# JacobPorter/FastNeighborNet

Measured on AMD Instinct MI355X. Metric: sec to circular order, n=32768 taxa (+ achieved HBM GB/s), lower is better.
Workload: dtype f64

## Files before the change

fastneighbornet_amd/csrc/fnn_hip.hip:

```cpp
#include <hip/hip_runtime.h>

#include <dlfcn.h>

#include <cmath>
#include <limits>
#include <new>

#include "fnn_chain.h"
#include "fnn_engine.h"

namespace fnn {

struct fnn_nccl_id { char internal[FNN_COMM_ID_BYTES]; };

constexpr int SCAN_TW = 512;
constexpr int SCAN_TH = 32;
constexpr int SCAN_THREADS = 256;

static_assert(sizeof(Cand) == 24, "rec_publish / rec_fetch move a Cand as three 8-byte words");
__device__ inline uint64_t rec_check_word(const Cand& c, uint32_t tag) {
    return __builtin_bit_cast(uint64_t, c.q) ^ (c.key * 0x9E3779B97F4A7C15ULL) ^
           ((uint64_t)(uint32_t)c.si | ((uint64_t)(uint32_t)c.sj << 32)) ^ (((uint64_t)tag + 1ULL) * 0xBF58476D1CE4E5B9ULL);
}
__device__ inline void rec_publish(Cand* p, const Cand& c, uint64_t* chk, uint32_t tag) {
    __hip_atomic_store(chk, rec_check_word(c, tag), __ATOMIC_RELAXED, __HIP_MEMORY_SCOPE_AGENT);
    uint64_t* w = (uint64_t*)p;
    __hip_atomic_store(w + 0, __builtin_bit_cast(uint64_t, c.q), __ATOMIC_RELAXED, __HIP_MEMORY_SCOPE_AGENT);
    __hip_atomic_store(w + 1, c.key, __ATOMIC_RELAXED, __HIP_MEMORY_SCOPE_AGENT);
    __hip_atomic_store(w + 2, (uint64_t)(uint32_t)c.si | ((uint64_t)(uint32_t)c.sj << 32), __ATOMIC_RELAXED, __HIP_MEMORY_SCOPE_AGENT);
}
__device__ inline Cand rec_fetch(const Cand* p) {
    uint64_t* w = (uint64_t*)p;
    const uint64_t a = __hip_atomic_load(w + 0, __ATOMIC_RELAXED, __HIP_MEMORY_SCOPE_AGENT);
    const uint64_t b = __hip_atomic_load(w + 1, __ATOMIC_RELAXED, __HIP_MEMORY_SCOPE_AGENT);
    const uint64_t x = __hip_atomic_load(w + 2, __ATOMIC_RELAXED, __HIP_MEMORY_SCOPE_AGENT);
    Cand c;
    c.q = __builtin_bit_cast(double, a);
    c.key = b;
    c.si = (int)(uint32_t)x;
    c.sj = (int)(uint32_t)(x >> 32);
    return c;
}

template <int CTRL, int ROW_MASK>
__device__ __forceinline__ void dpp_pull(double q, uint64_t key, double& oq, uint64_t& ok) {
    const uint64_t qb = __builtin_bit_cast(uint64_t, q);
    const int ql = (int)(uint32_t)qb, qh = (int)(uint32_t)(qb >> 32), kl = (int)(uint32_t)key, kh = (int)(uint32_t)(key >> 32);
    const uint32_t oql = (uint32_t)__builtin_amdgcn_update_dpp(ql, ql, CTRL, ROW_MASK, 0xf, false);
    const uint32_t oqh = (uint32_t)__builtin_amdgcn_update_dpp(qh, qh, CTRL, ROW_MASK, 0xf, false);
    const uint32_t okl = (uint32_t)__builtin_amdgcn_update_dpp(kl, kl, CTRL, ROW_MASK, 0xf, false);
    const uint32_t okh = (uint32_t)__builtin_amdgcn_update_dpp(kh, kh, CTRL, ROW_MASK, 0xf, false);
    oq = __builtin_bit_cast(double, ((uint64_t)oqh << 32) | oql);
    ok = ((uint64_t)okh << 32) | okl;
}
__device__ __forceinline__ Cand wave_reduce(Cand c) {
    double q = c.q;
    uint64_t key = c.key;
#define FNN_DPP_STEP(CTRL, MASK) do { double oq; uint64_t ok; dpp_pull<CTRL, MASK>(q, key, oq, ok); \
        if (oq < q || (oq == q && ok < key)) { q = oq; key = ok; } } while (0)
    FNN_DPP_STEP(0x111, 0xf);
    FNN_DPP_STEP(0x112, 0xf);
    FNN_DPP_STEP(0x114, 0xf);
    FNN_DPP_STEP(0x118, 0xf);
    FNN_DPP_STEP(0x142, 0xa);
    FNN_DPP_STEP(0x143, 0xc);
#undef FNN_DPP_STEP
    Cand r;
    const uint64_t qb = __builtin_bit_cast(uint64_t, q);
    const uint32_t rql = (uint32_t)__builtin_amdgcn_readlane((int)(uint32_t)qb, 63), rqh = (uint32_t)__builtin_amdgcn_readlane((int)(uint32_t)(qb >> 32), 63);
    const uint32_t rkl = (uint32_t)__builtin_amdgcn_readlane((int)(uint32_t)key, 63), rkh = (uint32_t)__builtin_amdgcn_readlane((int)(uint32_t)(key >> 32), 63);
    r.q = __builtin_bit_cast(double, ((uint64_t)rqh << 32) | rql);
    r.key = ((uint64_t)rkh << 32) | rkl;
    const unsigned long long src = __ballot(c.key == r.key);
    const int l = src ? (int)__builtin_ctzll(src) : 0;
    r.si = __builtin_amdgcn_readlane(c.si, l);
    r.sj = __builtin_amdgcn_readlane(c.sj, l);
    return r;
}

template <int NWAVES>
__device__ __forceinline__ Cand block_reduce(Cand c, Cand* sh) {
    c = wave_reduce(c);
    int lane = threadIdx.x & 63, w = threadIdx.x >> 6;
    if (lane == 0) sh[w] = c;
    __syncthreads();
    if (threadIdx.x == 0) {
#pragma unroll
        for (int k = 1; k < NWAVES; k++)
            if (cand_better(sh[k], c)) c = sh[k];
    }
    return c;
}

constexpr int SCAN_R = SCAN_TW / SCAN_TH;

// ... 1895 lines not shown
            rl_rowmin_block(d, L);
            if (threadIdx.x == 0) rl_publish_part(d, L, seq);
        }
        return;
    }
    if (threadIdx.x < 64) {
        RlBlockEnv env{L, (int)threadIdx.x};
        const Cand out = relaxed_find(d, env);
        if (threadIdx.x == 0) {
            d.recs[0] = out;
            L.cmd = 2;
            if (gridDim.x > 1) st_sc1(d.rl_mail, rl_cmd_word(stamp, L.seq + 1u, RL_EXIT));
        }
        if (ticks && threadIdx.x == 0) {
            d.ticks[24] += L.tk[0]; d.ticks[25] += L.tk[1]; d.ticks[26] += (long long)wall_clock64() - tstart; d.ticks[27] += L.tk[3];
        }
        __syncthreads();
    } else {
        for (;;) {
            __syncthreads();
            if (L.cmd == 2) break;
            rl_rowmin_block(d, L);
        }
    }
}

template <bool HELP>
__global__ __launch_bounds__(CH_T) void k_decide(Dev d, const Cand* src, int nrecs, unsigned jobtag) {
    __shared__ ChainLds<CH_EPT> L;
    __shared__ DecideLds S;
    __shared__ Cand shc[CH_T / 64];
    __shared__ unsigned hword;
    State* st = d.st;
    if (HELP && blockIdx.x > 0) {
        rx_helper_workgroup(d, L, (int)blockIdx.x - 1, jobtag, &hword);
        return;
    }
    if (st->stall || st->la_hit) {
        if (HELP && threadIdx.x == 0) job_post(d, jobtag, 0u);
        return;
    }
    state_in(S.lst, st);
    if (threadIdx.x == 0) S.tkon = 0;
    Cand best = reduce_records(d, src, st->rl_active ? 1 : nrecs, shc);
    __syncthreads();
    decide_step<HELP, false>(d, S, L, best, jobtag);
    __syncthreads();
    if (threadIdx.x == 0) S.lst.rl_active = 0;
    __syncthreads();
    state_out(st, S.lst);
}

constexpr int TRK_THREADS = 1024;
constexpr int TRK_GROUP = 16;
constexpr int TRK_FLAG = 32 * 65;
constexpr int TRK_BAD = 32 * 67;

__device__ __forceinline__ void chain_workgroup(const Dev& d, ChainLds<CH_EPT>& L) {
    State* st = d.st;
    if (!st->chain_pending) return;
    const int32_t cU = st->chain_U, cm = st->chain_m;
    const unsigned evtag = (unsigned)st->n_events;
    const double usx = block_chain_sum2<CH_EPT>(d.chain, cm, CH_GUARD_BITS, L, nullptr);
    if (threadIdx.x == 0) {
        __hip_atomic_store(reinterpret_cast<uint64_t*>(d.Sx + cU), __builtin_bit_cast(uint64_t, usx), __ATOMIC_RELAXED, __HIP_MEMORY_SCOPE_AGENT);
        __hip_atomic_store(reinterpret_cast<uint64_t*>(d.Sx + cU + 1), __builtin_bit_cast(uint64_t, usx), __ATOMIC_RELAXED, __HIP_MEMORY_SCOPE_AGENT);
        __hip_atomic_store(reinterpret_cast<uint64_t*>(&upre_behind_ticket(d)->usx), __builtin_bit_cast(uint64_t, usx), __ATOMIC_RELAXED, __HIP_MEMORY_SCOPE_AGENT);
        asm volatile("s_waitcnt vmcnt(0)" ::: "memory");
        __hip_atomic_store(d.ticket + TRK_FLAG, evtag, __ATOMIC_RELAXED, __HIP_MEMORY_SCOPE_AGENT);
    }
}

__device__ __forceinline__ void sweep_exact_item(const Dev& d, int64_t r, const TrackArgs& ta, Cand& bx) {
    const int32_t half = (ta.m + 1) / 2;
    const int32_t fi = ta.nf0 + (int32_t)(r / half), cp = (int32_t)(r % half);
    if (fi >= ta.nf) return;
    const int32_t f0 = fresh_slot(d, fi, ta.m);
    if (f0 < 0) return;
    const int32_t s2 = 2 * cp;
    if (s2 >= ta.m || s2 == f0) return;
    const double* F0 = d.D + (int64_t)f0 * d.ld + s2;
    const double* F1 = F0 + d.ld;
    const double a0 = F0[0], a1 = F0[1], b0 = F1[0], b1 = F1[1];
    if (f0 > s2)
        scan_micro(f0, s2, ta.m, ta.twoP, ta.cm2, a0, a1, b0, b1, d.Sx[f0], d.Sx[f0 + 1], d.spos[f0], d.spos[f0 + 1],
                   d.Sx[s2], d.Sx[s2 + 1], d.spos[s2], d.spos[s2 + 1], bx);
    else
        scan_micro(s2, f0, ta.m, ta.twoP, ta.cm2, a0, b0, a1, b1, d.Sx[s2], d.Sx[s2 + 1], d.spos[s2], d.spos[s2 + 1],
                   d.Sx[f0], d.Sx[f0 + 1], d.spos[f0], d.spos[f0 + 1], bx);
}

constexpr int TRK_REC_U = 1024;

struct SpecialOut { double val, tu, tv; };
__device__ __forceinline__ SpecialOut special_wave(const Dev& d, const State& lst, double* blk, double* sxl, double* tl, int32_t* berr, double* chain_dst) {
    const int lane = threadIdx.x & 63;
    const int nS = __builtin_amdgcn_readfirstlane(lst.nS);
    const int32_t Sl = lane < nS ? lst.S[lane < MAX_S ? lane : 0] : -1;
    const int m_old = __builtin_amdgcn_readfirstlane(lst.m_old), twoP_old = 2 * __builtin_amdgcn_readfirstlane(lst.P_old);
    const int m = __builtin_amdgcn_readfirstlane(lst.m), twoP = 2 * __builtin_amdgcn_readfirstlane(lst.P);
    const int xs = __builtin_amdgcn_readfirstlane(lst.xs), ys = __builtin_amdgcn_readfirstlane(lst.ys);
    const int U = __builtin_amdgcn_readfirstlane(lst.U), V = U + 1;
    const int nops = __builtin_amdgcn_readfirstlane(lst.nops), ev_finish = __builtin_amdgcn_readfirstlane(lst.ev_finish);
    const int32_t myspos = (Sl >= 0 && Sl < m) ? d.spos[Sl] : 0;
    auto ixu = [&](int slot) -> int {
        const unsigned long long b = __ballot(Sl == slot && Sl >= 0);
        return b ? (int)__builtin_ctzll(b) : -1;
    };
    auto ixl = [&](int32_t slot) -> int {
        int r = -1;
#pragma unroll
        for (int j = 0; j < MAX_S; j++) if (__builtin_amdgcn_readlane(Sl, j) == slot && slot >= 0) r = j;
        return r;
    };
    const int me = lane;
    const int pold = (Sl >= 0 && Sl < twoP_old) ? ixl(Sl ^ 1) : -1;
    const int pnew = (Sl >= 0 && Sl < twoP && !(Sl & 1)) ? ixl(Sl + 1) : -1;
    auto B = [&](int r, int c) -> double& { return blk[r * MAX_S + c]; };
    auto bad = [&]() { *berr = 13; };
    SpecialOut out{0.0, 0.0, 0.0};
    if (!ev_finish) {
        const bool sp = Sl >= 0 && Sl < twoP_old;
        const bool act = Sl >= 0 && Sl < m_old && Sl != xs && Sl != ys && !(sp && (Sl & 1));
        double sx = 0.0, sxn = 0.0, told0 = 0.0, told1 = 0.0;
        bool bystander = true;
        if (act) { sx = sxl[me]; if (sp) { if (pold < 0) bad(); else sxn = sxl[pold]; } }
#pragma unroll
        for (int q = 0; q < 2; q++) {
            const int t = q == 0 ? xs : ys;
            const int tn = t < twoP_old ? (t ^ 1) : -1;
            const int it = ixu(t), itn = tn >= 0 ? ixu(tn) : -1;
            if (it < 0 || (tn >= 0 && itn < 0)) { bad(); continue; }
            if (!act) continue;
            if (Sl == t || Sl == tn) { bystander = false; continue; }
            double v;
            if (!sp && tn < 0) { const double e = B(it, me); v = e; told0 += e; }
            else if (sp && tn < 0) { const double e0 = B(it, me), e1 = B(it, pold); v = (e0 + e1) / 2.0; told0 += e0; told1 += e1; }
            else if (!sp && tn >= 0) { const double e0 = B(it, me), f0 = B(itn, me); v = (e0 + f0) / 2.0; told0 += 0.5 * (e0 + f0); }
            else {
                const double e0 = B(it, me), f0 = B(itn, me), e1 = B(it, pold), f1 = B(itn, pold);
                v = (((e0 + f0) + e1) + f1) / 4.0;
                told0 += 0.5 * (e0 + f0); told1 += 0.5 * (e1 + f1);
            }
            sx -= v;
            sxn -= v;
// ... 117 lines not shown
            const int32_t it = q == 0 ? pv.ix : pv.iy, itn = q == 0 ? pv.ixn : pv.iyn;
            const double me0 = it >= 0 ? e[it] : 0.0, mf0 = itn >= 0 ? e[itn] : 0.0;
            const double oe = __shfl_xor(me0, 1, 64), of = __shfl_xor(mf0, 1, 64);
            const double e0 = odd ? oe : me0, f0 = odd ? of : mf0, e1 = odd ? me0 : oe, f1 = odd ? mf0 : of;
            double v;
            if (!paired && itn < 0) { v = me0; told += me0; }
            else if (paired && itn < 0) { v = (e0 + e1) / 2.0; told += me0; }
            else if (!paired && itn >= 0) { v = (me0 + mf0) / 2.0; told += 0.5 * (me0 + mf0); }
            else { v = (((e0 + f0) + e1) + f1) / 4.0; told += 0.5 * (me0 + mf0); }
            sx -= v;
        }
    }
    double nv[MAX_TGT];
    double um = 0.0, vm = 0.0;
#pragma unroll
    for (int t = 0; t < MAX_TGT; t++) {
        nv[t] = 0.0;
        if (t < pv.ntgt) {
            nv[t] = tgt_eval(pv, t, [&](int32_t i) { return e[i]; });
            if (t == pv.tU) um = nv[t];
            if (t == pv.tV) vm = nv[t];
        }
    }
    if (act) {
        const int64_t rk = (int64_t)k * d.ld;
#pragma unroll
        for (int t = 0; t < MAX_TGT; t++) {
            if (t < pv.ntgt) {
                const int32_t dst = pv.tdst[t];
                const int64_t rb = (int64_t)dst * d.ld;
                d.D[rb + k] = nv[t];
                d.D[rk + dst] = nv[t];
                if (d.H) d.H[k < dst ? (int64_t)dst * d.ldh + k : (int64_t)k * d.ldh + dst] = bf16_from_double(nv[t]);
            }
        }
    }
    if (!pv.ev_finish) {
        const double uo = __shfl_xor(um, 1, 64), vo = __shfl_xor(vm, 1, 64);
        const double u0 = odd ? uo : um, v0 = odd ? vo : vm, u1 = odd ? um : uo, v1 = odd ? vm : vo;
        const double dpu = paired ? (((u0 + v0) + u1) + v1) / 4.0 : (um + vm) / 2.0;
        if (act) {
            const bool rep = !paired || !odd;
            d.Sx[k] = sx + dpu;
            chain_dst[chain_addr(pos)] = rep ? dpu : 0.0;
            d.T[k] = (t_old - told) + 0.5 * (um + vm);
            dsum = rep ? dpu : 0.0;
            dabs = dsum < 0.0 ? -dsum : dsum;
            tu = paired ? 0.5 * um : um;
            tv = paired ? 0.5 * vm : vm;
        }
    }
}

template <bool HELP>
__global__ __launch_bounds__(TRK_THREADS) void k_track(Dev d, int force_base, int timed, int has_scan, int tgroup, int ticks, unsigned jobtag) {
    __shared__ ChainLds<CH_EPT> L;
    __shared__ DecideLds S;
    __shared__ Cand sh[TRK_THREADS / 64], shu[TRK_THREADS / 64];
    __shared__ int lastflag;
    __shared__ double shs[2];
    __shared__ unsigned hword;
    State* st = d.st;
    if (blockIdx.x == 0) {
        chain_workgroup(d, L);
        return;
    }
    const int wg = (int)blockIdx.x - 1, G = (int)gridDim.x - 1 - (HELP ? TRK_NHELP : 0);
    if (HELP && wg >= G) {
        rx_helper_workgroup(d, L, wg - G, jobtag, &hword);
        return;
    }
    const bool prof = ticks != 0 && threadIdx.x == 0;
#define TRK_TICK(slot) do { if (prof) S.tk[(slot) + 1] = (long long)wall_clock64(); } while (0)
    if (threadIdx.x == 0) S.tkon = ticks;
    if (prof) S.tk[0] = (long long)wall_clock64();
    const int64_t start = (int64_t)wg * TRK_THREADS + threadIdx.x;
    PairRec rec0;
    rec0.wa = rec0.wb = 0; rec0.sa = rec0.sb = -1;
    rec0.e[0] = rec0.e[1] = rec0.e[2] = rec0.e[3] = 0.0;
    if (start < LA_PCAP) rec0 = track_pair_load(d, start);
    if (st->done) {
        if (wg == 0 && threadIdx.x == 0) {
            st->ev_active = 0;
            if (HELP) job_post(d, jobtag, 0u);
        }
        return;
    }
    state_in(S.lst, st);
    if (!has_scan && st->stall) {
        if (wg == 0 && threadIdx.x == 0) {
            st->n_stalled++;
            if (HELP) job_post(d, jobtag, 0u);
        }
        return;
    }
    if (force_base || !la_active(*st)) {
        if (wg == 0 && threadIdx.x == 0) {
            if (HELP) job_post(d, jobtag, 0u);
            st->ev_timed = timed;
            if (st->la_valid) st->la_prev_end = 0;
            la_prepare_base(*st, d.lacnt);
            st->stall = has_scan ? 0 : 1;
            if (!has_scan) st->n_stalled++;
        }
        return;
    }
    const int32_t chain_pending0 = st->chain_pending, chain_U0 = st->chain_U;
    const unsigned evtag0 = (unsigned)st->n_events;
    TrackArgs ta = track_args(*st);
    const int64_t items = track_item_count(ta);
    double eps_u = 0.0;
    bool giveup = false;
    const bool pending = chain_pending0 != 0 && ta.nf > ta.nf0;
    if (pending && ta.nf - ta.nf0 != 1) giveup = true;
    const bool approx = pending && !giveup;
    double2 up0 = make_double2(0.0, 0.0), up1 = up0, up2 = up0;
    const int npart = approx ? st->upart_n : 0;
    if (threadIdx.x < 64) {
        const double2* up = reinterpret_cast<const double2*>(d.upart);
        if ((int)threadIdx.x < npart) up0 = up[2 * threadIdx.x];
        if ((int)threadIdx.x + 64 < npart) up1 = up[2 * (threadIdx.x + 64)];
        if ((int)threadIdx.x + 128 < npart) up2 = up[2 * (threadIdx.x + 128)];
    }
    Cand best, bestu;
    best = cand_none();
    bestu = best;
    const int64_t stride = (int64_t)G * TRK_THREADS;
    TRK_TICK(0);
    if (start < ta.np) track_pair_rec(d, rec0, ta, best);
    for (int64_t it = start + stride; it < ta.np; it += stride) track_pair_item(d, it, ta, best);
    TRK_TICK(1);
    if (approx) {
        if (threadIdx.x < 64) {
            double su = (up0.x + up1.x) + up2.x, sa = (up0.y + up1.y) + up2.y;
            for (int b = threadIdx.x + 192; b < npart; b += 64) { su += d.upart[4 * b]; sa += d.upart[4 * b + 1]; }
#pragma unroll
            for (int off = 32; off >= 1; off >>= 1) { su += __shfl_down(su, off, 64); sa += __shfl_down(sa, off, 64); }
            if (threadIdx.x == 0) { shs[0] = su; shs[1] = sa; }
        }
        __syncthreads();
        ta.approx = 1;
        ta.usl = chain_U0;
        ta.sxu = shs[0];
        eps_u = 4.0 * ((double)ta.m + 8.0) * 1.1102230246251565e-16 * shs[1];
    }
    bool swept_ok = true;
    if (!giveup)
        for (int64_t r = stride - 1 - start; r < items - ta.np; r += stride) swept_ok = track_sweep_item(d, r, ta, best, bestu) && swept_ok;
    if (!swept_ok) atomicOr(d.ticket + TRK_BAD, 1u);
    TRK_TICK(2);
    {
        best = wave_reduce(best);
        if (ta.approx) bestu = wave_reduce(bestu);
        const int lane_ = threadIdx.x & 63, w_ = threadIdx.x >> 6;
        if (lane_ == 0) { sh[w_] = best; shu[w_] = bestu; }
        __syncthreads();
        if (w_ == 0) {
            Cand b2, bu2;
            b2 = cand_none(); bu2 = b2;
            if (lane_ < TRK_THREADS / 64) { b2 = sh[lane_]; bu2 = shu[lane_]; }
            best = wave_reduce(b2);
            if (ta.approx) bestu = wave_reduce(bu2);
            if (lane_ == 0) {
                rec_publish(&d.recs[wg], best, d.rchk + wg, evtag0);
                if (ta.approx) rec_publish(&d.recs[TRK_REC_U + wg], bestu, d.rchk + TRK_REC_U + wg, evtag0);
            }
        }
    }
    TRK_TICK(3);
    if (threadIdx.x == 0) {
        __builtin_amdgcn_s_waitcnt(0);
        const unsigned g = (unsigned)wg / (unsigned)tgroup, ngroups = ((unsigned)G + tgroup - 1) / (unsigned)tgroup;
        const unsigned gsize = g + 1 < ngroups ? (unsigned)tgroup : (unsigned)G - g * tgroup;
        int last = 0;
        if (atomicAdd(d.ticket + 32 * (g + 1), 1u) == gsize - 1) {
            d.ticket[32 * (g + 1)] = 0u;
            last = atomicAdd(d.ticket, 1u) == ngroups - 1 ? 1 : 0;
        }
        lastflag = last;
    }
    __syncthreads();
    if (!lastflag) return;
    TRK_TICK(4);
    State& lst = S.lst;
    Dev dl = d;
    dl.st = &lst;
    if (threadIdx.x < 64) {
        Cand b, bu;
        b = cand_none();
        bu = b;
        const unsigned badword = __hip_atomic_load(d.ticket + TRK_BAD, __ATOMIC_RELAXED, __HIP_MEMORY_SCOPE_AGENT);
        const uint32_t tag = evtag0;
        bool stale = false, reread = false;
        for (int pass = 0; pass < 2; pass++) {
            b = cand_none();
            bu = b;
            stale = false;
            for (int i = threadIdx.x; i < G; i += 64) {
                Cand c = rec_fetch(&d.recs[i]);
                if (rec_check_word(c, tag) != __hip_atomic_load(d.rchk + i, __ATOMIC_RELAXED, __HIP_MEMORY_SCOPE_AGENT)) stale = true;
                if (cand_better(c, b)) b = c;
                if (ta.approx) {
                    c = rec_fetch(&d.recs[TRK_REC_U + i]);
                    if (rec_check_word(c, tag) != __hip_atomic_load(d.rchk + TRK_REC_U + i, __ATOMIC_RELAXED, __HIP_MEMORY_SCOPE_AGENT)) stale = true;
                    if (cand_better(c, bu)) bu = c;
                }
            }
            stale = __ballot(stale) != 0ULL;
            if (!stale) break;
            reread = true;
            __threadfence();
        }
        b = wave_reduce(b);
        if (ta.approx) bu = wave_reduce(bu);
        if (threadIdx.x == 0) {
            sh[0] = b;
            shu[0] = bu;
            if (badword != 0u) {
                d.ticket[TRK_BAD] = 0u;
                lastflag = 2;
            }
            if (stale) lastflag = 2;
            if (reread) S.lst.n_ev_persistent++;
        }
    }
    __syncthreads();
    best = sh[0];
    bestu = shu[0];
    if (lastflag == 2) {
        giveup = true;
        if (d.strict && threadIdx.x == 0) S.lst.error = 13;
    }
    __syncthreads();
    TRK_TICK(5);
    if (ta.approx && !giveup) {
        const double dmax = __builtin_bit_cast(double, lst.dmax_bits);
        const double margin = 2.0 * eps_u + 192.0 * 1.1102230246251565e-16 * ((double)lst.n + 4.0) * dmax + 1e-300;
        const bool certain = (bestu.q - margin > best.q) || (bestu.q == inf_f64());
        if (!certain) {
            if (threadIdx.x == 0) {
                const unsigned want = evtag0;
                const long long t_wait = (long long)wall_clock64();
                while (__hip_atomic_load(d.ticket + TRK_FLAG, __ATOMIC_RELAXED, __HIP_MEMORY_SCOPE_AGENT) != want) {
                    if ((long long)wall_clock64() - t_wait > TRK_WAIT_TICKS) { lst.error = 10; break; }
                    __builtin_amdgcn_s_sleep(2);
                }
                __threadfence();
                lst.n_sweep_waits++;
            }
            __syncthreads();
            Cand bx;
            bx = cand_none();
            for (int64_t r = threadIdx.x; r < items - ta.np; r += TRK_THREADS) sweep_exact_item(d, r, ta, bx);
            bx = block_reduce<TRK_THREADS / 64>(bx, sh);
            if (threadIdx.x == 0) sh[0] = bx;
            __syncthreads();
            bx = sh[0];
            if (cand_better(bx, best)) best = bx;
        }
    }
    if (giveup) { best = cand_none(); }
    if (threadIdx.x == 0) {
        *d.ticket = 0u;
        lst.ev_timed = timed;
        if (giveup) lst.n_sweep_waits++;
        la_track_done(dl, best, ta);
        lst.stall = (!lst.la_hit && !has_scan) ? 1 : 0;
        if (lst.stall) lst.n_stalled++;
    }
    __syncthreads();
    TRK_TICK(6);
    if (lst.la_hit) decide_step<HELP, true>(d, S, L, best, jobtag);
    else if (HELP && threadIdx.x == 0) job_post(d, jobtag, 0u);
    TRK_TICK(7);
    if (prof) {
        for (int q = 0; q < 8; q++) d.ticks[q] += S.tk[q + 1] - S.tk[q];
    }
    __syncthreads();
    state_out(st, lst);
#undef TRK_TICK
}


struct FeedArg {
    FeedRec* box;
    int64_t seq;
    int32_t gen;
};
__device__ __forceinline__ void feed_post(const FeedArg& f, const State& st) {
    if (!f.box) return;
    const FeedWords w = feed_record(st, f.gen, f.seq);
    uint64_t* dst = reinterpret_cast<uint64_t*>(f.box + (int)(f.seq & (FEED_RING - 1)));
#pragma unroll
    for (int k = 0; k < FEED_WORDS; k++) __hip_atomic_store(dst + k, w.w[k], __ATOMIC_RELAXED, __HIP_MEMORY_SCOPE_SYSTEM);
}
static_assert((FEED_RING & (FEED_RING - 1)) == 0, "the ring's slot is the low bits of the sequence number");

__global__ __launch_bounds__(256) void k_update(Dev d, int defer, int ticks, FeedArg feed) {
    __shared__ double shp[4][4];
    __shared__ State lst;
    State* st = d.st;
    const bool special = blockIdx.x == gridDim.x - 1;
    const UpdPlan pl = d.upre->plan;
    const int32_t g_active = st->ev_active, g_stall = st->stall, g_u_id = st->cur.u_id;
    long long tk0 = 0;
    const bool prof = ticks != 0 && threadIdx.x == 0 && (special || blockIdx.x == 0);
    const int tkb = special ? 0 : 4;
#define UPD_TICK(slot) do { if (prof) { const long long now_ = (long long)wall_clock64(); d.ticks[8 + tkb + (slot)] += now_ - tk0; tk0 = now_; } } while (0)
    if (prof) tk0 = (long long)wall_clock64();
    const long long wg_t0 = (ticks != 0 && threadIdx.x == 0) ? (long long)wall_clock64() : 0;
    double dsum = 0.0, dabs = 0.0, tu = 0.0, tv = 0.0;
    if (!special) {
        if (!g_active || g_stall || pl.u_id != g_u_id) return;
        UPD_TICK(0);
        const PlanView pv = upd_plan_view(pl);
        UPD_TICK(1);
        bulk_column(d, pv, (int32_t)(blockIdx.x * 256 + threadIdx.x), d.chain, dsum, dabs, tu, tv);
        UPD_TICK(2);
    } else {
        __shared__ double blk[MAX_S * MAX_S], sxl[MAX_S], tl[MAX_S];
        __shared__ int32_t berr;
        UpdPre* const up = d.upre;
        const int t = (int)threadIdx.x;
        double pre = 0.0;
        if (t < MAX_S * MAX_S) pre = up->blk[t];
        else if (t < MAX_S * MAX_S + MAX_S) pre = up->sxl[t - MAX_S * MAX_S];
        else if (t < MAX_S * MAX_S + 2 * MAX_S) pre = up->tl[t - MAX_S * MAX_S - MAX_S];
        const int64_t pevent = up->event;
        const int32_t pu_id = up->u_id, pmask = up->mask;
// ... 198 lines not shown
}

#define HIPOK(x) ((last = (x)) == hipSuccess)

struct HipBackend {
    static constexpr int64_t kRowPad = SCAN_TH;
    static constexpr int64_t kColPad = SCR_TW;
    int32_t screen_min_n() const { int32_t v = 4096; env_int("FNN_SCREEN_MIN_N", 8, INT_MAX, &v); return v; }
    int screen_min_m = 2048;
    bool screen_min_m_fixed = false;
    int relaxed_grid = 0;
    int relaxed_min = 0;
    void set_relaxed(int32_t min_active) { relaxed_min = min_active; }
    void set_problem_size(int32_t n) {
        if (screen_min_m_fixed) return;
        const int v = n / 4;
        screen_min_m = v < 512 ? 512 : (v > 2048 ? 2048 : v);
    }
    hipError_t last = hipSuccess;
    hipStream_t stream = nullptr;
    int device = 0;
    bool opened = false;
    int timing = 0;
    double class_ms[16] = {0};
    int64_t class_n[16] = {0};
    std::vector<hipEvent_t> ev_pool;
    std::vector<char> ev_kind;
    size_t ev_used = 0;
    double scan_ms = 0.0, plain_ms = 0.0;
    int64_t scan_launches = 0, plain_launches = 0;
    int* d_bad = nullptr;
    double* d_stage = nullptr;
    int64_t stage_cap = 0;
    void* rccl_lib = nullptr;
    void* rccl_comm = nullptr;
    int (*p_ncclCommInitRank)(void**, int, fnn_nccl_id, int) = nullptr;
    int (*p_ncclAllGather)(const void*, void*, size_t, int, void*, hipStream_t) = nullptr;
    int (*p_ncclCommDestroy)(void*) = nullptr;
    const char* (*p_ncclGetErrorString)(int) = nullptr;
    std::string comm_err;
    int scan_grid = 8192;
    int unsched_grid = 2048;
    int emit_grid = 256;
    int track_grid = 64;
    int rx_helpers_cfg = TRK_NHELP;
    int rx_helpers = 0;
    int64_t rx_exact_seen = 0;
    void note_rx_exact(int64_t n_rx_exact) {
        rx_helpers = n_rx_exact > rx_exact_seen ? rx_helpers_cfg : 0;
        rx_exact_seen = n_rx_exact;
    }
    unsigned track_tag = 0;
    bool unsched_scans = false;
    int track_group = TRK_GROUP;
    bool defer_chain = false;
    bool scan_nt = true;
    bool ticks = false;

    std::string err() const { return comm_err.empty() ? std::string(hipGetErrorString(last)) : comm_err; }

    static void* open_rccl(const char* path, std::string& why) {
        const char* cands[4] = {path, path && *path ? nullptr : std::getenv("FNN_RCCL_PATH"), path && *path ? nullptr : "librccl.so.1",
                                path && *path ? nullptr : "librccl.so"};
        for (const char* c : cands) {
            if (!c || !*c) continue;
            if (void* h = dlopen(c, RTLD_NOW | RTLD_LOCAL)) return h;
            why = dlerror();
        }
        return nullptr;
    }
    int32_t comm_init_rccl(int world, int rank, const uint8_t* id, const char* path) {
        comm_err.clear();
        if (!rccl_lib && !(rccl_lib = open_rccl(path, comm_err))) { comm_err = "cannot load librccl: " + comm_err; return FNN_ERCCL; }
        p_ncclCommInitRank = (decltype(p_ncclCommInitRank))dlsym(rccl_lib, "ncclCommInitRank");
        p_ncclAllGather = (decltype(p_ncclAllGather))dlsym(rccl_lib, "ncclAllGather");
        p_ncclCommDestroy = (decltype(p_ncclCommDestroy))dlsym(rccl_lib, "ncclCommDestroy");
        p_ncclGetErrorString = (decltype(p_ncclGetErrorString))dlsym(rccl_lib, "ncclGetErrorString");
        if (!p_ncclCommInitRank || !p_ncclAllGather || !p_ncclCommDestroy) { comm_err = "librccl lacks the expected symbols"; return FNN_ERCCL; }
        fnn_nccl_id uid;
        std::memcpy(uid.internal, id, sizeof(uid.internal));
        (void)hipSetDevice(device);
        int rc = p_ncclCommInitRank(&rccl_comm, world, uid, rank);
        if (rc != 0) rccl_comm = nullptr;
        return rc == 0 ? FNN_OK : nccl_failed("ncclCommInitRank", rc);
    }
    int32_t nccl_failed(const char* call, int rc) {
        comm_err = std::string(call) + ": " + (p_ncclGetErrorString ? p_ncclGetErrorString(rc) : "error");
        return FNN_ERCCL;
    }
    int32_t allgather_bytes_on_stream(const void* send, void* recv, size_t bytes) {
        if (!rccl_comm) { comm_err = "RCCL communicator not initialised"; return FNN_ERCCL; }
        const int rc = p_ncclAllGather(send, recv, bytes,  0, rccl_comm, stream);
        return rc == 0 ? FNN_OK : nccl_failed("ncclAllGather", rc);
    }
    int32_t allgather_wx_on_stream(const Dev& d, size_t bytes) {
        int32_t rc = FNN_ERCCL;
        timed(TC_GATHER, timing == 2 && rccl_comm != nullptr, [&] { rc = allgather_bytes_on_stream(d.wsend, d.wrecv, bytes); });
        return rc;
    }

    int32_t open(int32_t dev) {
        int cnt = 0;
        if (!HIPOK(hipGetDeviceCount(&cnt)) || cnt <= 0)
            return fail(FNN_EHIP, "no HIP device available (" + err() + ")");
        if (dev < 0 || dev >= cnt) return fail(FNN_EINVAL, "device ordinal out of range");
        device = dev;
        if (!HIPOK(hipSetDevice(device))) return fail(FNN_EHIP, "hipSetDevice failed (" + err() + ")");
        if (!HIPOK(hipStreamCreateWithFlags(&stream, hipStreamNonBlocking)))
            return fail(FNN_EHIP, "hipStreamCreate failed (" + err() + ")");
        bool help = true;
        env_int("FNN_SCAN_GRID", 1, 65535, &scan_grid);
        env_flag("FNN_SCAN_NT", &scan_nt);
        env_flag("FNN_TICKS", &ticks);
        env_int("FNN_UNSCHED_GRID", 1, 65535, &unsched_grid);
        env_flag("FNN_UNSCHED_SCANS", &unsched_scans);
        env_int("FNN_EMIT_GRID", 1, 65535, &emit_grid);
        if (env_flag("FNN_RX_HELPERS", &help)) rx_helpers_cfg = help ? TRK_NHELP : 0;
        env_int("FNN_TRACK_GROUP", 2, 1024, &track_group);
        env_int("FNN_TRACK_GRID", 1, 1024, &track_grid);
        static_assert(TRK_FLAG == 32 * 65 && TRK_BAD == 32 * 67, "ticket layout: groups 1..64, then the flag words");
        while ((track_grid + track_group - 1) / track_group > 64) track_group *= 2;
        env_int("FNN_RELAXED_GRID", 1, RL_GMAX, &relaxed_grid);
        screen_min_m_fixed = env_int("FNN_SCREEN_MIN_M", 8, INT_MAX, &screen_min_m);
        if (hipHostMalloc((void**)&box, sizeof(FeedRec) * FEED_RING, hipHostMallocMapped | hipHostMallocCoherent) != hipSuccess) {
            (void)hipGetLastError();
            box = nullptr;
        }
        if (box && hipHostGetDevicePointer((void**)&box_dev, box, 0) != hipSuccess) {
            (void)hipGetLastError();
            (void)hipHostFree(box);
            box = nullptr;
        }
        opened = true;
        return FNN_OK;
    }
    void close() {
        if (!opened) return;
        (void)hipSetDevice(device);
        if (rccl_comm && p_ncclCommDestroy) (void)p_ncclCommDestroy(rccl_comm);
        rccl_comm = nullptr;
        for (hipEvent_t e : ev_pool) (void)hipEventDestroy(e);
        ev_pool.clear();
        if (d_bad) (void)hipFree(d_bad);
        d_bad = nullptr;
        if (d_stage) (void)hipFree(d_stage);
        d_stage = nullptr;
        stage_cap = 0;
        if (stream) (void)hipStreamSynchronize(stream);
        if (box) (void)hipHostFree(box);
        box = box_dev = nullptr;
        feed_on = false;
        if (stream) (void)hipStreamDestroy(stream);
        stream = nullptr;
        opened = false;
    }
    void* alloc(size_t b) {
        void* p = nullptr;
        (void)hipSetDevice(device);
        if (!HIPOK(hipMalloc(&p, b ? b : 8))) {
            (void)hipGetLastError();
            (void)fnn_split_weights_release_cache();
            if (!HIPOK(hipMalloc(&p, b ? b : 8))) return nullptr;
        }
        return p;
    }
    void free(void* p) {
        if (p) (void)hipFree(p);
    }
    size_t max_records(int32_t) { return 65536; }
    int32_t memset(void* p, int v, size_t b) {
        return HIPOK(hipMemsetAsync(p, v, b, stream)) && HIPOK(hipStreamSynchronize(stream)) ? FNN_OK : FNN_EHIP;
    }
    int32_t h2d(void* d, const void* s, size_t b) {
        return HIPOK(hipMemcpyAsync(d, s, b, hipMemcpyHostToDevice, stream)) && HIPOK(hipStreamSynchronize(stream)) ? FNN_OK : FNN_EHIP;
// ... 73 lines not shown
        }
        return ev_pool[ev_used++];
    }

    static dim3 grid1(int32_t cnt) { return dim3((unsigned)((cnt + 255) / 256 > 0 ? (cnt + 255) / 256 : 1)); }

    int32_t launch_synth(const Dev& d, uint64_t seed, int32_t dist) {
        dim3 g((unsigned)((d.n + 255) / 256), (unsigned)d.n);
        launch(TC_OTHER, false, k_synth, g, dim3(256), d, seed, dist);
        return launched_and_done();
    }
    int32_t unpack_rows(const Dev& d, const double* src, int64_t p0, int64_t entries, int32_t row0, int32_t cnt) {
        if (entries > stage_cap) {
            if (d_stage) (void)hipFree(d_stage);
            d_stage = nullptr;
            stage_cap = 0;
            if (!HIPOK(hipMalloc((void**)&d_stage, sizeof(double) * (size_t)entries))) return FNN_EHIP;
            stage_cap = entries;
        }
        if (!HIPOK(hipMemcpyAsync(d_stage, src, sizeof(double) * (size_t)entries, hipMemcpyHostToDevice, stream))) return FNN_EHIP;
        dim3 g((unsigned)((d.n + 255) / 256), (unsigned)cnt);
        launch(TC_OTHER, false, k_unpack, g, dim3(256), d, (const double*)d_stage, p0, row0);
        return launched_and_done();
    }
    int32_t launch_mirror(const Dev& d) {
        if (d_stage) (void)hipFree(d_stage);
        d_stage = nullptr;
        stage_cap = 0;
        unsigned t = (unsigned)((d.n + 31) / 32);
        launch(TC_OTHER, false, k_mirror, dim3(t, t), dim3(256), d);
        return launched_and_done();
    }
    int32_t launch_validate(const Dev& d, int32_t* bad) {
        if (!d_bad && !HIPOK(hipMalloc((void**)&d_bad, sizeof(int)))) return FNN_EHIP;
        if (!HIPOK(hipMemsetAsync(d_bad, 0, sizeof(int), stream))) return FNN_EHIP;
        unsigned t = (unsigned)((d.n + 31) / 32);
        launch(TC_OTHER, false, k_validate, dim3(t, t), dim3(256), d, d_bad);
        if (launched() != FNN_OK) return FNN_EHIP;
        int hb = 0;
        if (!HIPOK(hipMemcpyAsync(&hb, d_bad, sizeof(int), hipMemcpyDeviceToHost, stream)) ||
            !HIPOK(hipStreamSynchronize(stream)))
            return FNN_EHIP;
        *bad = hb;
        return FNN_OK;
    }
    int32_t launch_prep_screen(const Dev& d, int64_t nrows) {
        const int64_t want = (nrows * d.ld + 255) / 256;
        launch(TC_OTHER, false, k_prep_screen, dim3((unsigned)(want < 8192 ? (want > 0 ? want : 1) : 8192)), dim3(256), d, nrows);
        return launched();
    }
    int32_t launch_init(const Dev& d) {
        reset_timing();
        rx_exact_seen = 0; rx_helpers = 0;
        launch(TC_OTHER, false, k_init, grid1(d.n), dim3(256), d);
        return launched();
    }

    dim3 scan_dims(const Dev& d, int32_t m_bound) const {
        int nt = (scan_tile_count(m_bound) + d.world - 1) / d.world;
        return dim3((unsigned)(nt < scan_grid ? (nt > 0 ? nt : 1) : scan_grid));
    }
    bool screen_off = false;
    bool keep_generic_screen() const { return false; }
    bool use_screen(const Dev& d, int32_t m_bound) const { return d.H != nullptr && !screen_off && m_bound >= screen_min_m; }
    int enqueue_scan(const Dev& d, int32_t m_bound, bool sched) {
        const bool screen = use_screen(d, m_bound);
        const bool tscan = timing != 0 && (sched || !screen), tall = timing == 2;
        const bool has_scan = sched || !screen || unsched_scans;
        if (d.la) {
            const bool help = rx_helpers > 0;
            const int fb = (sched || !screen) ? 1 : 0, hs = has_scan ? 1 : 0, tk = ticks ? 1 : 0;
            track_tag = (track_tag % 0x7FFFFFEu) + 1u;
            const int tgrid = fb ? 1 : track_grid;
            launch(TC_TRACK, tall, help ? k_track<true> : k_track<false>, dim3(tgrid + 1 + (help ? TRK_NHELP : 0)), dim3(TRK_THREADS),
                   d, fb, fb, hs, track_group, tk, track_tag);
        }
        if (screen && !has_scan) return 0;
        if (screen) {
            static constexpr decltype(&k_screen<true, true>) variants[2][2] = {{k_screen<true, true>, k_screen<false, true>},
                                                                               {k_screen<true, false>, k_screen<false, false>}};
            int nt = (tri_tile_count(m_bound, SCR_TH, SCR_R) + d.world - 1) / d.world;
            const int want = sched ? scan_grid : unsched_grid;
            launch(TC_SCREEN, tscan, variants[!sched][!scan_nt], dim3((unsigned)(nt < want ? (nt > 0 ? nt : 1) : want)), dim3(256), d);
            if (d.la) launch(TC_EMIT, tall, k_emit, dim3(emit_grid), dim3(256), d);
            launch(TC_RESOLVE, tall, k_resolve, dim3(RES_BLOCKS), dim3(1024), d);
            if (tscan) scan_launches++;
            return RES_BLOCKS;
        }
        if (relaxed_min > 0 && m_bound > relaxed_min) {
            int g = relaxed_grid > 0 ? relaxed_grid : (m_bound >= 12288 ? m_bound / 4096 : 1);
            launch(TC_OTHER, tall, k_relaxed, dim3(g > RL_GMAX ? RL_GMAX : g), dim3(RL_T), d, ticks ? 1 : 0);
        }
        const dim3 gs = scan_dims(d, m_bound);
        launch(TC_SCAN, tscan, scan_nt ? k_scan<true> : k_scan<false>, gs, dim3(SCAN_THREADS), d);
        if (tscan) plain_launches++;
        return (int)gs.x;
    }
    void enqueue_rest(const Dev& d, int32_t m_bound, const Cand* src, int nrecs) {
        const bool tall = timing == 2, help = rx_helpers > 0;
        if (nrecs > 0) {
            track_tag = (track_tag % 0x7FFFFFEu) + 1u;
            launch(TC_DECIDE, tall, help ? k_decide<true> : k_decide<false>, dim3(1 + (help ? TRK_NHELP : 0)), dim3(CH_T), d, src, nrecs, track_tag);
        }
        const FeedArg feed{feed_on ? box_dev : nullptr, feed_on ? feed_seq++ : 0, feed_gen};
        launch(TC_UPDATE, tall, k_update, dim3(grid1(m_bound).x + 1), dim3(256), d, defer_chain ? 1 : 0, ticks ? 1 : 0, feed);
        if (!defer_chain) launch(TC_OTHER, tall, k_finalize, dim3(1), dim3(CH_T), d, feed);
    }
    FeedRec* box = nullptr;
    FeedRec* box_dev = nullptr;
    bool feed_on = false;
    int32_t feed_gen = 0;
    int64_t feed_seq = 0;
    bool feed_begin(int64_t first_seq) {
        if (!box || !HIPOK(hipStreamSynchronize(stream))) return false;
        feed_gen = feed_gen == INT32_MAX ? 1 : feed_gen + 1;
        std::memset(box, 0, sizeof(FeedRec) * FEED_RING);
        feed_seq = first_seq;
        feed_on = true;
        return true;
    }
    void feed_end() { feed_on = false; }
    bool feed_timing_ok() const { return timing != 2; }
    bool feed_newest(int64_t seen, FeedRec* out) const { return feed_pick(box, FEED_RING, feed_gen, seen, out); }
    int32_t feed_wait(int64_t seen, FeedRec* out, double limit_s) {
        const double t0 = now_s();
        double asked = t0;
        for (int64_t spins = 1;; spins++) {
            if (feed_newest(seen, out)) return FNN_OK;
// ... 357 lines not shown
```

Baseline: 1.257.

## Replace track ticket counters with dedicated decider block polling tagged granules

The tracking kernel used to finish with a two-level atomic ticket counter, where the last-arriving workgroup fetched all per-workgroup records and checked them against checksums. That is replaced by a dedicated decider block. Each worker publishes its best candidate as tag-stamped 32-bit words in a per-workgroup line, and the decider polls those lines in parallel across waves until every tag matches. This removes the atomic counter chain and the checksum re-read pass from the critical path. In exchange it spends one whole workgroup spinning, adds a timeout path that reports error 10, and needs a memset of the granule lines at init.

```diff
diff --git a/fastneighbornet_amd/csrc/fnn_hip.hip b/fastneighbornet_amd/csrc/fnn_hip.hip
--- a/fastneighbornet_amd/csrc/fnn_hip.hip
+++ b/fastneighbornet_amd/csrc/fnn_hip.hip
@@ -16,31 +16,6 @@
 constexpr int SCAN_TW = 512;
 constexpr int SCAN_TH = 32;
 constexpr int SCAN_THREADS = 256;
-
-static_assert(sizeof(Cand) == 24, "rec_publish / rec_fetch move a Cand as three 8-byte words");
-__device__ inline uint64_t rec_check_word(const Cand& c, uint32_t tag) {
-    return __builtin_bit_cast(uint64_t, c.q) ^ (c.key * 0x9E3779B97F4A7C15ULL) ^
-           ((uint64_t)(uint32_t)c.si | ((uint64_t)(uint32_t)c.sj << 32)) ^ (((uint64_t)tag + 1ULL) * 0xBF58476D1CE4E5B9ULL);
-}
-__device__ inline void rec_publish(Cand* p, const Cand& c, uint64_t* chk, uint32_t tag) {
-    __hip_atomic_store(chk, rec_check_word(c, tag), __ATOMIC_RELAXED, __HIP_MEMORY_SCOPE_AGENT);
-    uint64_t* w = (uint64_t*)p;
-    __hip_atomic_store(w + 0, __builtin_bit_cast(uint64_t, c.q), __ATOMIC_RELAXED, __HIP_MEMORY_SCOPE_AGENT);
-    __hip_atomic_store(w + 1, c.key, __ATOMIC_RELAXED, __HIP_MEMORY_SCOPE_AGENT);
-    __hip_atomic_store(w + 2, (uint64_t)(uint32_t)c.si | ((uint64_t)(uint32_t)c.sj << 32), __ATOMIC_RELAXED, __HIP_MEMORY_SCOPE_AGENT);
-}
-__device__ inline Cand rec_fetch(const Cand* p) {
-    uint64_t* w = (uint64_t*)p;
-    const uint64_t a = __hip_atomic_load(w + 0, __ATOMIC_RELAXED, __HIP_MEMORY_SCOPE_AGENT);
-    const uint64_t b = __hip_atomic_load(w + 1, __ATOMIC_RELAXED, __HIP_MEMORY_SCOPE_AGENT);
-    const uint64_t x = __hip_atomic_load(w + 2, __ATOMIC_RELAXED, __HIP_MEMORY_SCOPE_AGENT);
-    Cand c;
-    c.q = __builtin_bit_cast(double, a);
-    c.key = b;
-    c.si = (int)(uint32_t)x;
-    c.sj = (int)(uint32_t)(x >> 32);
-    return c;
-}
 
 template <int CTRL, int ROW_MASK>
 __device__ __forceinline__ void dpp_pull(double q, uint64_t key, double& oq, uint64_t& ok) {
@@ -2042,9 +2017,38 @@
 }
 
 constexpr int TRK_THREADS = 1024;
-constexpr int TRK_GROUP = 16;
 constexpr int TRK_FLAG = 32 * 65;
 constexpr int TRK_BAD = 32 * 67;
+
+constexpr int TRK_GRAN_REC0 = 32768;
+constexpr int TRK_GRAN_LINE = 16;
+constexpr int TRK_GRAN_TICK = 12;
+constexpr int TRK_GRID_MAX = 1024;
+static_assert((TRK_GRAN_REC0 * sizeof(Cand)) % 128 == 0, "granule lines are 128-byte aligned within d.recs");
+static_assert(TRK_GRAN_REC0 * sizeof(Cand) + (size_t)TRK_GRID_MAX * TRK_GRAN_LINE * 8 <= 65536 * sizeof(Cand), "granule lines end inside d.recs (HipBackend::max_records)");
+__host__ __device__ __forceinline__ uint64_t* trk_line(const Dev& d, int wg) {
+    return reinterpret_cast<uint64_t*>(d.recs + TRK_GRAN_REC0) + (size_t)wg * TRK_GRAN_LINE;
+}
+__device__ __forceinline__ void gran_store(uint64_t* g, uint32_t payload, unsigned tag) {
+    __hip_atomic_store(g, (uint64_t)payload | ((uint64_t)tag << 32), __ATOMIC_RELAXED, __HIP_MEMORY_SCOPE_AGENT);
+}
+__device__ __forceinline__ void gran_publish(uint64_t* g, const Cand& c, unsigned tag) {
+    const uint64_t qb = __builtin_bit_cast(uint64_t, c.q);
+    gran_store(g + 0, (uint32_t)qb, tag);
+    gran_store(g + 1, (uint32_t)(qb >> 32), tag);
+    gran_store(g + 2, (uint32_t)c.key, tag);
+    gran_store(g + 3, (uint32_t)(c.key >> 32), tag);
+    gran_store(g + 4, (uint32_t)c.si, tag);
+    gran_store(g + 5, (uint32_t)c.sj, tag);
+}
+__device__ __forceinline__ Cand gran_cand(uint32_t (*pay)[64], int set, int lane) {
+    Cand c;
+    c.q = __builtin_bit_cast(double, (uint64_t)pay[6 * set][lane] | ((uint64_t)pay[6 * set + 1][lane] << 32));
+    c.key = (uint64_t)pay[6 * set + 2][lane] | ((uint64_t)pay[6 * set + 3][lane] << 32);
+    c.si = (int)pay[6 * set + 4][lane];
+    c.sj = (int)pay[6 * set + 5][lane];
+    return c;
+}
 
 __device__ __forceinline__ void chain_workgroup(const Dev& d, ChainLds<CH_EPT>& L) {
     State* st = d.st;
@@ -2079,8 +2083,6 @@
         scan_micro(s2, f0, ta.m, ta.twoP, ta.cm2, a0, b0, a1, b1, d.Sx[s2], d.Sx[s2 + 1], d.spos[s2], d.spos[s2 + 1],
                    d.Sx[f0], d.Sx[f0 + 1], d.spos[f0], d.spos[f0 + 1], bx);
 }
-
-constexpr int TRK_REC_U = 1024;
 
 struct SpecialOut { double val, tu, tv; };
 __device__ __forceinline__ SpecialOut special_wave(const Dev& d, const State& lst, double* blk, double* sxl, double* tl, int32_t* berr, double* chain_dst) {
@@ -2304,12 +2306,75 @@
     }
 }
 
+__device__ __forceinline__ void trk_gather(const Dev& d, int G, unsigned tag, int nw, uint32_t (*pay)[64], int* wlate, Cand* sh, Cand* shu,
+                                        int* flag, int* late_out, long long* tk) {
+    const int lane = threadIdx.x & 63, w = threadIdx.x >> 6;
+    const bool two = nw > 6;
+    Cand b, bu;
+    b = cand_none();
+    bu = b;
+    int late = 0;
+    const long long t0 = (long long)wall_clock64();
+    for (int c0 = 0; c0 < G; c0 += 64) {
+        if (w < nw) {
+            const bool live = c0 + lane < G;
+            const uint64_t* g = trk_line(d, live ? c0 + lane : 0) + w;
+            uint64_t x;
+            for (;;) {
+                x = __hip_atomic_load(g, __ATOMIC_RELAXED, __HIP_MEMORY_SCOPE_AGENT);
+                if (__all(!live || (unsigned)(x >> 32) == tag)) break;
+                if ((long long)wall_clock64() - t0 > TRK_WAIT_TICKS) { late = 1; break; }
+                __builtin_amdgcn_s_sleep(1);
+            }
+            pay[w][lane] = (uint32_t)x;
+            if (lane == 0) wlate[w] = late;
+        }
+        __syncthreads();
+        if (tk && threadIdx.x == 0 && c0 + 64 >= G) tk[0] = (long long)wall_clock64();
+        if (w == 0 && c0 + lane < G) {
+            const Cand c = gran_cand(pay, 0, lane);
+            if (cand_better(c, b)) b = c;
+            if (two) {
+                const Cand cu = gran_cand(pay, 1, lane);
+                if (cand_better(cu, bu)) bu = cu;
+            }
+        }
+        if (c0 + 64 < G) __syncthreads();
+    }
+    if (w == 0) {
+        b = wave_reduce(b);
+        if (two) bu = wave_reduce(bu);
+        if (lane == 0) {
+            const unsigned badword = __hip_atomic_load(d.ticket + TRK_BAD, __ATOMIC_RELAXED, __HIP_MEMORY_SCOPE_AGENT);
+            int anylate = 0;
+            for (int k = 0; k < nw; k++) anylate |= wlate[k];
+            sh[0] = b;
+            shu[0] = bu;
+            if (badword != 0u) d.ticket[TRK_BAD] = 0u;
+            *flag = (badword != 0u || anylate) ? 2 : 1;
+            *late_out = anylate;
+            if (tk) {
+                uint64_t x = 0;
+                if (!anylate) {
+                    const uint64_t* g = trk_line(d, G - 1) + TRK_GRAN_TICK;
+                    do x = __hip_atomic_load(g, __ATOMIC_RELAXED, __HIP_MEMORY_SCOPE_AGENT);
+                    while ((unsigned)(x >> 32) != tag && (long long)wall_clock64() - t0 <= TRK_WAIT_TICKS);
+                }
+                tk[2] = (unsigned)(x >> 32) == tag ? tk[0] - (long long)(int32_t)((uint32_t)tk[0] - (uint32_t)x) : tk[0];
+            }
+        }
+    }
+    __syncthreads();
+    if (tk && threadIdx.x == 0) tk[1] = (long long)wall_clock64();
+}
+
 template <bool HELP>
-__global__ __launch_bounds__(TRK_THREADS) void k_track(Dev d, int force_base, int timed, int has_scan, int tgroup, int ticks, unsigned jobtag) {
+__global__ __launch_bounds__(TRK_THREADS) void k_track(Dev d, int force_base, int timed, int has_scan, int ticks, unsigned jobtag) {
     __shared__ ChainLds<CH_EPT> L;
     __shared__ DecideLds S;
     __shared__ Cand sh[TRK_THREADS / 64], shu[TRK_THREADS / 64];
-    __shared__ int lastflag;
+    __shared__ int lastflag, lateflag, wlate[12];
+    __shared__ uint32_t pay[12][64];
     __shared__ double shs[2];
     __shared__ unsigned hword;
     State* st = d.st;
@@ -2317,37 +2382,38 @@
         chain_workgroup(d, L);
         return;
     }
-    const int wg = (int)blockIdx.x - 1, G = (int)gridDim.x - 1 - (HELP ? TRK_NHELP : 0);
+    const int wg = (int)blockIdx.x - 2, G = (int)gridDim.x - 2 - (HELP ? TRK_NHELP : 0);
     if (HELP && wg >= G) {
         rx_helper_workgroup(d, L, wg - G, jobtag, &hword);
         return;
     }
-    const bool prof = ticks != 0 && threadIdx.x == 0;
+    const bool decider = blockIdx.x == 1;
+    const bool prof = ticks != 0 && threadIdx.x == 0 && (decider || wg == G - 1);
 #define TRK_TICK(slot) do { if (prof) S.tk[(slot) + 1] = (long long)wall_clock64(); } while (0)
-    if (threadIdx.x == 0) S.tkon = ticks;
+    if (decider && threadIdx.x == 0) S.tkon = ticks;
     if (prof) S.tk[0] = (long long)wall_clock64();
     const int64_t start = (int64_t)wg * TRK_THREADS + threadIdx.x;
     PairRec rec0;
     rec0.wa = rec0.wb = 0; rec0.sa = rec0.sb = -1;
     rec0.e[0] = rec0.e[1] = rec0.e[2] = rec0.e[3] = 0.0;
-    if (start < LA_PCAP) rec0 = track_pair_load(d, start);
+    if (!decider && start < LA_PCAP) rec0 = track_pair_load(d, start);
     if (st->done) {
-        if (wg == 0 && threadIdx.x == 0) {
+        if (decider && threadIdx.x == 0) {
             st->ev_active = 0;
             if (HELP) job_post(d, jobtag, 0u);
         }
         return;
     }
-    state_in(S.lst, st);
+    if (decider) state_in(S.lst, st);
     if (!has_scan && st->stall) {
-        if (wg == 0 && threadIdx.x == 0) {
+        if (decider && threadIdx.x == 0) {
             st->n_stalled++;
             if (HELP) job_post(d, jobtag, 0u);
         }
         return;
     }
     if (force_base || !la_active(*st)) {
-        if (wg == 0 && threadIdx.x == 0) {
+        if (decider && threadIdx.x == 0) {
             if (HELP) job_post(d, jobtag, 0u);
             st->ev_timed = timed;
             if (st->la_valid) st->la_prev_end = 0;
@@ -2379,8 +2445,10 @@
     bestu = best;
     const int64_t stride = (int64_t)G * TRK_THREADS;
     TRK_TICK(0);
-    if (start < ta.np) track_pair_rec(d, rec0, ta, best);
-    for (int64_t it = start + stride; it < ta.np; it += stride) track_pair_item(d, it, ta, best);
+    if (!decider) {
+        if (start < ta.np) track_pair_rec(d, rec0, ta, best);
+        for (int64_t it = start + stride; it < ta.np; it += stride) track_pair_item(d, it, ta, best);
+    }
     TRK_TICK(1);
     if (approx) {
         if (threadIdx.x < 64) {
@@ -2396,12 +2464,15 @@
         ta.sxu = shs[0];
         eps_u = 4.0 * ((double)ta.m + 8.0) * 1.1102230246251565e-16 * shs[1];
     }
-    bool swept_ok = true;
-    if (!giveup)
-        for (int64_t r = stride - 1 - start; r < items - ta.np; r += stride) swept_ok = track_sweep_item(d, r, ta, best, bestu) && swept_ok;
-    if (!swept_ok) atomicOr(d.ticket + TRK_BAD, 1u);
-    TRK_TICK(2);
-    {
+    if (!decider) {
+        bool swept_ok = true;
+        if (!giveup)
+            for (int64_t r = stride - 1 - start; r < items - ta.np; r += stride) swept_ok = track_sweep_item(d, r, ta, best, bestu) && swept_ok;
+        if (!swept_ok) {
+            __hip_atomic_store(d.ticket + TRK_BAD, 1u, __ATOMIC_RELAXED, __HIP_MEMORY_SCOPE_AGENT);
+            __builtin_amdgcn_s_waitcnt(0);
+        }
+        TRK_TICK(2);
         best = wave_reduce(best);
         if (ta.approx) bestu = wave_reduce(bestu);
         const int lane_ = threadIdx.x & 63, w_ = threadIdx.x >> 6;
@@ -2414,77 +2485,33 @@
             best = wave_reduce(b2);
             if (ta.approx) bestu = wave_reduce(bu2);
             if (lane_ == 0) {
-                rec_publish(&d.recs[wg], best, d.rchk + wg, evtag0);
-                if (ta.approx) rec_publish(&d.recs[TRK_REC_U + wg], bestu, d.rchk + TRK_REC_U + wg, evtag0);
-            }
-        }
-    }
-    TRK_TICK(3);
-    if (threadIdx.x == 0) {
-        __builtin_amdgcn_s_waitcnt(0);
-        const unsigned g = (unsigned)wg / (unsigned)tgroup, ngroups = ((unsigned)G + tgroup - 1) / (unsigned)tgroup;
-        const unsigned gsize = g + 1 < ngroups ? (unsigned)tgroup : (unsigned)G - g * tgroup;
-        int last = 0;
-        if (atomicAdd(d.ticket + 32 * (g + 1), 1u) == gsize - 1) {
-            d.ticket[32 * (g + 1)] = 0u;
-            last = atomicAdd(d.ticket, 1u) == ngroups - 1 ? 1 : 0;
-        }
-        lastflag = last;
-    }
-    __syncthreads();
-    if (!lastflag) return;
-    TRK_TICK(4);
+                uint64_t* g = trk_line(d, wg);
+                const long long t_store = prof ? (long long)wall_clock64() : 0;
+                gran_publish(g, best, jobtag);
+                if (ta.approx) gran_publish(g + 6, bestu, jobtag);
+                if (prof) {
+                    gran_store(g + TRK_GRAN_TICK, (uint32_t)t_store, jobtag);
+                    S.tk[4] = t_store;
+                    for (int q = 0; q < 4; q++) d.ticks[q] += S.tk[q + 1] - S.tk[q];
+                }
+            }
+        }
+        return;
+    }
     State& lst = S.lst;
     Dev dl = d;
     dl.st = &lst;
-    if (threadIdx.x < 64) {
-        Cand b, bu;
-        b = cand_none();
-        bu = b;
-        const unsigned badword = __hip_atomic_load(d.ticket + TRK_BAD, __ATOMIC_RELAXED, __HIP_MEMORY_SCOPE_AGENT);
-        const uint32_t tag = evtag0;
-        bool stale = false, reread = false;
-        for (int pass = 0; pass < 2; pass++) {
-            b = cand_none();
-            bu = b;
-            stale = false;
-            for (int i = threadIdx.x; i < G; i += 64) {
-                Cand c = rec_fetch(&d.recs[i]);
-                if (rec_check_word(c, tag) != __hip_atomic_load(d.rchk + i, __ATOMIC_RELAXED, __HIP_MEMORY_SCOPE_AGENT)) stale = true;
-                if (cand_better(c, b)) b = c;
-                if (ta.approx) {
-                    c = rec_fetch(&d.recs[TRK_REC_U + i]);
-                    if (rec_check_word(c, tag) != __hip_atomic_load(d.rchk + TRK_REC_U + i, __ATOMIC_RELAXED, __HIP_MEMORY_SCOPE_AGENT)) stale = true;
-                    if (cand_better(c, bu)) bu = c;
-                }
-            }
-            stale = __ballot(stale) != 0ULL;
-            if (!stale) break;
-            reread = true;
-            __threadfence();
-        }
-        b = wave_reduce(b);
-        if (ta.approx) bu = wave_reduce(bu);
-        if (threadIdx.x == 0) {
-            sh[0] = b;
-            shu[0] = bu;
-            if (badword != 0u) {
-                d.ticket[TRK_BAD] = 0u;
-                lastflag = 2;
-            }
-            if (stale) lastflag = 2;
-            if (reread) S.lst.n_ev_persistent++;
-        }
-    }
-    __syncthreads();
+    trk_gather(d, G, jobtag, approx ? 12 : 6, pay, wlate, sh, shu, &lastflag, &lateflag, ticks ? &S.tk[5] : nullptr);
     best = sh[0];
     bestu = shu[0];
     if (lastflag == 2) {
         giveup = true;
-        if (d.strict && threadIdx.x == 0) S.lst.error = 13;
-    }
-    __syncthreads();
-    TRK_TICK(5);
+        if (threadIdx.x == 0) {
+            if (lateflag) S.lst.error = 10;
+            else if (d.strict) S.lst.error = 13;
+        }
+    }
+    __syncthreads();
     if (ta.approx && !giveup) {
         const double dmax = __builtin_bit_cast(double, lst.dmax_bits);
         const double margin = 2.0 * eps_u + 192.0 * 1.1102230246251565e-16 * ((double)lst.n + 4.0) * dmax + 1e-300;
@@ -2513,7 +2540,6 @@
     }
     if (giveup) { best = cand_none(); }
     if (threadIdx.x == 0) {
-        *d.ticket = 0u;
         lst.ev_timed = timed;
         if (giveup) lst.n_sweep_waits++;
         la_track_done(dl, best, ta);
@@ -2521,12 +2547,15 @@
         if (lst.stall) lst.n_stalled++;
     }
     __syncthreads();
-    TRK_TICK(6);
+    TRK_TICK(7);
     if (lst.la_hit) decide_step<HELP, true>(d, S, L, best, jobtag);
     else if (HELP && threadIdx.x == 0) job_post(d, jobtag, 0u);
-    TRK_TICK(7);
+    TRK_TICK(8);
     if (prof) {
-        for (int q = 0; q < 8; q++) d.ticks[q] += S.tk[q + 1] - S.tk[q];
+        d.ticks[4] += S.tk[5] - S.tk[7];
+        d.ticks[5] += S.tk[6] - S.tk[5];
+        d.ticks[6] += S.tk[8] - S.tk[6];
+        d.ticks[7] += S.tk[9] - S.tk[8];
     }
     __syncthreads();
     state_out(st, lst);
@@ -2831,7 +2860,6 @@
     }
     unsigned track_tag = 0;
     bool unsched_scans = false;
-    int track_group = TRK_GROUP;
     bool defer_chain = false;
     bool scan_nt = true;
     bool ticks = false;
@@ -2888,17 +2916,14 @@
         if (!HIPOK(hipStreamCreateWithFlags(&stream, hipStreamNonBlocking)))
             return fail(FNN_EHIP, "hipStreamCreate failed (" + err() + ")");
         bool help = true;
-        env_int("FNN_SCAN_GRID", 1, 65535, &scan_grid);
+        env_int("FNN_SCAN_GRID", 1, TRK_GRAN_REC0, &scan_grid);
         env_flag("FNN_SCAN_NT", &scan_nt);
         env_flag("FNN_TICKS", &ticks);
         env_int("FNN_UNSCHED_GRID", 1, 65535, &unsched_grid);
         env_flag("FNN_UNSCHED_SCANS", &unsched_scans);
         env_int("FNN_EMIT_GRID", 1, 65535, &emit_grid);
         if (env_flag("FNN_RX_HELPERS", &help)) rx_helpers_cfg = help ? TRK_NHELP : 0;
-        env_int("FNN_TRACK_GROUP", 2, 1024, &track_group);
-        env_int("FNN_TRACK_GRID", 1, 1024, &track_grid);
-        static_assert(TRK_FLAG == 32 * 65 && TRK_BAD == 32 * 67, "ticket layout: groups 1..64, then the flag words");
-        while ((track_grid + track_group - 1) / track_group > 64) track_group *= 2;
+        env_int("FNN_TRACK_GRID", 1, TRK_GRID_MAX, &track_grid);
         env_int("FNN_RELAXED_GRID", 1, RL_GMAX, &relaxed_grid);
         screen_min_m_fixed = env_int("FNN_SCREEN_MIN_M", 8, INT_MAX, &screen_min_m);
         if (hipHostMalloc((void**)&box, sizeof(FeedRec) * FEED_RING, hipHostMallocMapped | hipHostMallocCoherent) != hipSuccess) {
@@ -3078,6 +3103,7 @@
     int32_t launch_init(const Dev& d) {
         reset_timing();
         rx_exact_seen = 0; rx_helpers = 0;
+        if (d.recs && !HIPOK(hipMemsetAsync(trk_line(d, 0), 0, (size_t)TRK_GRID_MAX * TRK_GRAN_LINE * sizeof(uint64_t), stream))) return FNN_EHIP;
         launch(TC_OTHER, false, k_init, grid1(d.n), dim3(256), d);
         return launched();
     }
@@ -3097,9 +3123,9 @@
             const bool help = rx_helpers > 0;
             const int fb = (sched || !screen) ? 1 : 0, hs = has_scan ? 1 : 0, tk = ticks ? 1 : 0;
             track_tag = (track_tag % 0x7FFFFFEu) + 1u;
-            const int tgrid = fb ? 1 : track_grid;
-            launch(TC_TRACK, tall, help ? k_track<true> : k_track<false>, dim3(tgrid + 1 + (help ? TRK_NHELP : 0)), dim3(TRK_THREADS),
-                   d, fb, fb, hs, track_group, tk, track_tag);
+            const int tgrid = fb ? 0 : track_grid;
+            launch(TC_TRACK, tall, help ? k_track<true> : k_track<false>, dim3(tgrid + 2 + (help ? TRK_NHELP : 0)), dim3(TRK_THREADS),
+                   d, fb, fb, hs, tk, track_tag);
         }
         if (screen && !has_scan) return 0;
         if (screen) {
```

New measurement: 1.251 (median of 6 runs). About the same (-0.5%).
